# michal-szadkowski/rl-selfplay-mnk

Measured on AMD Instinct MI355X. Metric: env-steps/sec 9x9x5, 65536 parallel envs/GPU, random-policy rollout, higher is better.
Workload: dtype u64

## Files before the change

### rl-selfplay-mnk_amd/csrc/mnk_device.h

```cpp
#pragma once
#ifdef __HIPCC_RTC__
typedef unsigned char uint8_t;
typedef unsigned short uint16_t;
typedef unsigned int uint32_t;
typedef unsigned long long uint64_t;
typedef signed char int8_t;
typedef int int32_t;
typedef long long int64_t;
typedef unsigned long long uintptr_t;
#include "mnk_hip.h"
#else
#include <hip/hip_runtime.h>
#include <stdint.h>

#include "../../include/mnk_hip.h"
#endif

#define MNK_MAX_W 16
#define MNK_MAX_NW 32

struct MnkGeom {
  int m, n, k;
  int C;
  int W;
  int NW;
  int stride;
  uint32_t magic_n;
  uint32_t magic_stride;
  uint32_t magic_C;
  uint32_t magic_2C;
  uint32_t valid[MNK_MAX_NW];
};

__device__ __forceinline__ uint32_t mnk_div(uint32_t x, uint32_t magic) { return __umulhi(x, magic); }

__host__ __device__ inline bool aligned16(const void* p) { return (((uintptr_t)p) & 15u) == 0; }

struct MnkSample {
  const void* logits;
  int logits_dtype;
  const uint8_t* mask;
  uint64_t seed;
  const uint64_t* seed_dev;
  uint64_t step;
  const uint64_t* step_dev;
  int64_t env_id0;
  int deterministic;
  int64_t* actions;
  float* logp;
};

template <int CN>
__device__ __forceinline__ int geom_n(const MnkGeom& g) { return CN ? CN : g.n; }
template <int CK>
__device__ __forceinline__ int geom_k(const MnkGeom& g) { return CK ? CK : g.k; }

template <int CN>
__device__ __forceinline__ int mnk_bit_cell(const MnkGeom& g, uint32_t bit) {
  constexpr uint32_t magic = CN ? (uint32_t)((0x100000000ull + CN) / (uint32_t)(CN + 1)) : 0u;
  return (int)(bit - (CN ? __umulhi(bit, magic) : mnk_div(bit, g.magic_stride)));
}
template <int CN>
__device__ __forceinline__ uint32_t mnk_cell_bit(const MnkGeom& g, uint32_t cell) {
  return cell + (CN ? cell / (uint32_t)CN : mnk_div(cell, g.magic_n));
}

template <int NW>
__device__ __forceinline__ void bs_shr(uint32_t (&x)[NW], int s) {
  for (int q = s >> 5; q > 0; --q) {
#pragma unroll
    for (int w = 0; w < NW; ++w) x[w] = (w + 1 < NW) ? x[w + 1] : 0u;
  }
  const int r = s & 31;
  if (r) {
#pragma unroll
    for (int w = 0; w < NW; ++w) x[w] = __builtin_amdgcn_alignbit((w + 1 < NW) ? x[w + 1] : 0u, x[w], (uint32_t)r);
  }
}

template <int NW>
__device__ __forceinline__ void bs_shl(uint32_t (&x)[NW], int s) {
  for (int q = s >> 5; q > 0; --q) {
#pragma unroll
    for (int w = NW - 1; w >= 0; --w) x[w] = w > 0 ? x[w - 1] : 0u;
  }
  const int r = s & 31;
  if (r) {
#pragma unroll
    for (int w = NW - 1; w >= 0; --w) x[w] = __builtin_amdgcn_alignbit(x[w], w > 0 ? x[w - 1] : 0u, (uint32_t)(32 - r));
  }
}

template <int NW>
__device__ __forceinline__ bool bs_has_run(const uint32_t (&b)[NW], int d, int k) {
  uint32_t x[NW], t[NW];
#pragma unroll
  for (int w = 0; w < NW; ++w) x[w] = b[w];
  int len = 1;
  while (2 * len <= k) {
#pragma unroll
    for (int w = 0; w < NW; ++w) t[w] = x[w];
    bs_shr<NW>(t, len * d);
#pragma unroll
    for (int w = 0; w < NW; ++w) x[w] &= t[w];
    len *= 2;
  }
  if (len + 1 == k) {
#pragma unroll
    for (int w = 0; w < NW; ++w) t[w] = b[w];
    bs_shr<NW>(t, len * d);
#pragma unroll
    for (int w = 0; w < NW; ++w) x[w] &= t[w];
  } else if (len < k) {
#pragma unroll
    for (int w = 0; w < NW; ++w) t[w] = x[w];
    bs_shr<NW>(t, (k - len) * d);
#pragma unroll
    for (int w = 0; w < NW; ++w) x[w] &= t[w];
  }
  uint32_t any = 0;
#pragma unroll
  for (int w = 0; w < NW; ++w) any |= x[w];
  return any != 0;
}

template <int NW, int CN, int CK>
__device__ __forceinline__ bool mnk_plane_wins(const MnkGeom& g, const uint32_t (&b)[NW]) {
  const int n = geom_n<CN>(g), k = geom_k<CK>(g);
  bool hit = bs_has_run<NW>(b, 1, k);
  hit |= bs_has_run<NW>(b, n + 1, k);
  hit |= bs_has_run<NW>(b, n + 2, k);
  hit |= bs_has_run<NW>(b, n, k);
  return hit;
}

template <int NW, int CN, int CK>
__device__ __forceinline__ void mnk_plane_completions(const MnkGeom& g, const uint32_t (&plane)[NW],
                                                      const uint32_t (&empty)[NW], uint32_t (&out)[NW]) {
  const int n = geom_n<CN>(g), k = geom_k<CK>(g);
  constexpr int UK = CK ? CK : 1;
  uint32_t acc[NW];
#pragma unroll
  for (int w = 0; w < NW; ++w) acc[w] = 0u;
#pragma unroll
  for (int dir = 0; dir < 4; ++dir) {
    const int d = dir == 0 ? 1 : (dir == 1 ? n + 1 : (dir == 2 ? n + 2 : n));
    uint32_t lj[NW];
#pragma unroll
    for (int w = 0; w < NW; ++w) lj[w] = ~0u;
#pragma unroll UK
    for (int j = 0; j < k; ++j) {
      if (j > 0) {
        uint32_t t[NW];
#pragma unroll
        for (int w = 0; w < NW; ++w) t[w] = plane[w];
        bs_shl<NW>(t, j * d);
#pragma unroll
        for (int w = 0; w < NW; ++w) lj[w] &= t[w];
      }
      uint32_t rj[NW];
#pragma unroll
      for (int w = 0; w < NW; ++w) rj[w] = ~0u;
#pragma unroll UK
      for (int i = 1; i < k - j; ++i) {
        uint32_t t[NW];
#pragma unroll
        for (int w = 0; w < NW; ++w) t[w] = plane[w];
        bs_shr<NW>(t, i * d);
#pragma unroll
        for (int w = 0; w < NW; ++w) rj[w] &= t[w];
      }
#pragma unroll
      for (int w = 0; w < NW; ++w) acc[w] |= lj[w] & rj[w];
    }
  }
#pragma unroll
  for (int w = 0; w < NW; ++w) out[w] = acc[w] & empty[w];
}

#define MNK_SELECT_LEVEL(S)                        \
  "v_bfe_u32 %[t], %[x], %[pos], " #S "\n\t"       \
  "v_bcnt_u32_b32 %[t], %[t], %[nr]\n\t"          \
  "v_max_u32 %[nr], %[nr], %[t]\n\t"              \
  "v_ashrrev_i32 %[t], 31, %[t]\n\t"              \
  "v_and_or_b32 %[pos], %[t], " #S ", %[pos]\n\t"
__device__ __forceinline__ uint32_t select_bit32_nr(uint32_t x, uint32_t nr, uint32_t base) {
  uint32_t pos, t;
  asm("v_and_b32 %[t], 0xffff, %[x]\n\t"
      "v_bcnt_u32_b32 %[t], %[t], %[nr]\n\t"
      "v_max_u32 %[nr], %[nr], %[t]\n\t"
      "v_ashrrev_i32 %[t], 31, %[t]\n\t"
      "v_and_or_b32 %[pos], %[t], 16, %[base]\n\t"
      MNK_SELECT_LEVEL(8) MNK_SELECT_LEVEL(4) MNK_SELECT_LEVEL(2)
      "v_bfe_u32 %[t], %[x], %[pos], 1\n\t"
      "v_bitop3_b32 %[t], %[nr], %[t], %[t] bitop3:0x3f\n\t"
      "v_and_or_b32 %[pos], %[t], 1, %[pos]"
      : [pos] "=&v"(pos), [t] "=&v"(t), [nr] "+v"(nr)
      : [x] "v"(x), [base] "v"(base));
  return pos;
}
#undef MNK_SELECT_LEVEL

__device__ __forceinline__ int select_bit32(uint32_t x, int r) { return (int)select_bit32_nr(x, ~(uint32_t)r, 0u); }

template <int NW>
__device__ __forceinline__ int bs_popcount(const uint32_t (&x)[NW]) {
  int c = 0;
#pragma unroll
  for (int w = 0; w < NW; ++w) c += __popc(x[w]);
  return c;
}

template <int NW>
__device__ __forceinline__ int bs_select_hot(const uint32_t (&x)[NW], int r_, uint32_t (&hot)[NW]) {
  const uint32_t nr = ~(uint32_t)r_;
  uint32_t m[NW + 1], word = x[0], base = 0u, rank = nr, pre = 0u;
  m[0] = ~0u;
  m[NW] = 0u;
#pragma unroll
  for (int w = 1; w < NW; ++w) {
    pre += (uint32_t)__popc(x[w - 1]);
    const uint32_t t = pre + nr;
    m[w] = (uint32_t)((int32_t)t >> 31);
    rank = rank > t ? rank : t;
    word = __builtin_amdgcn_bitop3_b32(m[w], x[w], word, 0xca);
    base = __builtin_amdgcn_bitop3_b32(m[w], 32u * w, base, 0xca);
  }
  const uint32_t pos = select_bit32_nr(word, rank, base);
  const uint32_t one = 1u << (pos & 31u);
#pragma unroll
  for (int w = 0; w < NW; ++w) hot[w] = __builtin_amdgcn_bitop3_b32(one, m[w], m[w + 1], 0x40);
  return (int)pos;
}

template <int NW>
__device__ __forceinline__ int bs_select(const uint32_t (&x)[NW], int r) {
  uint32_t hot[NW];
  return bs_select_hot<NW>(x, r, hot);
}

struct Philox4 { uint32_t v[4]; };

__device__ __forceinline__ uint64_t mnk_mul_wide(uint32_t a, uint32_t m) {
  uint64_t product, carry;
  asm("v_mad_u64_u32 %0, %1, %2, %3, 0" : "=v"(product), "=s"(carry) : "v"(a), "s"(m));
  return product;
}

__device__ __forceinline__ Philox4 philox4x32_10(uint32_t c0, uint32_t c1, uint32_t c2, uint32_t c3,
                                                 uint32_t k0, uint32_t k1) {
  const uint32_t M0 = 0xD2511F53u, M1 = 0xCD9E8D57u;
#pragma unroll
  for (int r = 0; r < 10; ++r) {
    const uint64_t p0 = mnk_mul_wide(c0, M0), p1 = mnk_mul_wide(c2, M1);
    const uint32_t n0 = __builtin_amdgcn_bitop3_b32((uint32_t)(p1 >> 32), c1, k0, 0x96);
    const uint32_t n2 = __builtin_amdgcn_bitop3_b32((uint32_t)(p0 >> 32), c3, k1, 0x96);
    c0 = n0; c1 = (uint32_t)p1; c2 = n2; c3 = (uint32_t)p0;
    k0 += 0x9E3779B9u; k1 += 0xBB67AE85u;
  }
  Philox4 o;
  o.v[0] = c0; o.v[1] = c1; o.v[2] = c2; o.v[3] = c3;
  return o;
}

__device__ __forceinline__ Philox4 mnk_rng_block(uint64_t seed, uint64_t env, uint64_t q, uint32_t stream) {
  return philox4x32_10((uint32_t)env, (uint32_t)(env >> 32), (uint32_t)q,
                       stream | ((uint32_t)((q >> 32) & 0xFFFFFFu) << 8),
                       (uint32_t)seed, (uint32_t)(seed >> 32));
}

__device__ __forceinline__ uint32_t philox_word(const Philox4& b, uint32_t i) {
  uint32_t lo = (i & 1u) ? b.v[1] : b.v[0];
  uint32_t hi = (i & 1u) ? b.v[3] : b.v[2];
  return (i & 2u) ? hi : lo;
}

__device__ __forceinline__ uint32_t mnk_rand_u32(uint64_t seed, uint64_t env, uint64_t step, uint32_t stream) {
  Philox4 b = mnk_rng_block(seed, env, step >> 2, stream);
  return philox_word(b, (uint32_t)(step & 3));
}

template <int NW>
struct MnkEnv {
  uint32_t p[2][NW];
  uint32_t meta;
};

template <int NW, bool EXACT = false>
__device__ __forceinline__ void plane_load(uint32_t (&x)[NW], const uint64_t* plane, int64_t N, int W, int64_t i) {
#pragma unroll
  for (int q = 0; q < (NW + 1) / 2; ++q) {
    const uint64_t v = (EXACT || q < W) ? plane[(int64_t)q * N + i] : 0ull;
    x[2 * q] = (uint32_t)v;
    if (2 * q + 1 < NW) x[2 * q + 1] = (uint32_t)(v >> 32);
  }
}

template <int NW, bool EXACT = false>
__device__ __forceinline__ void plane_store(const uint32_t (&x)[NW], uint64_t* plane, int64_t N, int W, int64_t i) {
#pragma unroll
  for (int q = 0; q < (NW + 1) / 2; ++q) {
    const uint64_t hi = (2 * q + 1 < NW) ? (uint64_t)x[2 * q + 1] : 0ull;
    if (EXACT || q < W) plane[(int64_t)q * N + i] = (uint64_t)x[2 * q] | (hi << 32);
  }
}

template <int NW, bool EXACT = false>
__device__ __forceinline__ void rec_store(const uint32_t (&p0)[NW], const uint32_t (&p1)[NW], uint64_t* rows, int64_t N,
                                          int nw, int64_t i) {
#pragma unroll
  for (int w = 0; w < NW; ++w)
    if (EXACT || w < nw) rows[(int64_t)w * N + i] = (uint64_t)p0[w] | ((uint64_t)p1[w] << 32);
}

template <int NW, bool EXACT = false>
__device__ __forceinline__ void rec_load(uint32_t (&p0)[NW], uint32_t (&p1)[NW], const uint64_t* rows, int64_t N, int nw,
                                         int64_t i) {
#pragma unroll
  for (int w = 0; w < NW; ++w) {
    const uint64_t v = (EXACT || w < nw) ? rows[(int64_t)w * N + i] : 0ull;
    p0[w] = (uint32_t)v;
    p1[w] = (uint32_t)(v >> 32);
  }
}

template <int NW, bool EXACT = false>
__device__ __forceinline__ void env_load(MnkEnv<NW>& e, const uint64_t* planes, const uint32_t* meta, int64_t N,
                                         int W, int64_t i) {
  plane_load<NW, EXACT>(e.p[0], planes, N, W, i);
  plane_load<NW, EXACT>(e.p[1], planes + (int64_t)W * N, N, W, i);
  e.meta = meta[i];
}

template <int NW, bool EXACT = false>
__device__ __forceinline__ void env_store(const MnkEnv<NW>& e, uint64_t* planes, uint32_t* meta, int64_t N, int W,
                                          int64_t i) {
  plane_store<NW, EXACT>(e.p[0], planes, N, W, i);
  plane_store<NW, EXACT>(e.p[1], planes + (int64_t)W * N, N, W, i);
  meta[i] = e.meta;
}

template <int NW>
__device__ __forceinline__ void env_clear(MnkEnv<NW>& e) {
#pragma unroll
  for (int pl = 0; pl < 2; ++pl)
#pragma unroll
    for (int w = 0; w < NW; ++w) e.p[pl][w] = 0u;
  e.meta = 0u;
}

template <int NW>
__device__ __forceinline__ void env_legal(const MnkGeom& g, const MnkEnv<NW>& e, uint32_t (&legal)[NW]) {
#pragma unroll
  for (int w = 0; w < NW; ++w) legal[w] = ~(e.p[0][w] | e.p[1][w]) & g.valid[w];
}

template <int NW, int CN>
__device__ __forceinline__ int bs_pick_cell(const MnkGeom& g, uint32_t (&set)[NW], uint32_t x) {
  const int nl = bs_popcount<NW>(set);
#pragma unroll
  for (int w = 0; w < NW; ++w) set[w] = nl ? set[w] : g.valid[w];
  const int r = (int)__umulhi(x, (uint32_t)(nl ? nl : g.C));
  const uint32_t bit = (uint32_t)bs_select<NW>(set, r);
  return mnk_bit_cell<CN>(g, bit);
}

template <int NW, int CN>
__device__ __forceinline__ int env_pick_legal(const MnkGeom& g, const MnkEnv<NW>& e, uint32_t x) {
  uint32_t legal[NW];
  env_legal<NW>(g, e, legal);
  return bs_pick_cell<NW, CN>(g, legal, x);
}

template <int NW, int CN, int CK>
__device__ __forceinline__ void mnk_tactical_set(const MnkGeom& g, const uint32_t (&mine)[NW], const uint32_t (&theirs)[NW],
                                                 uint32_t (&set)[NW]) {
  uint32_t legal[NW], win[NW], block[NW];
#pragma unroll
  for (int w = 0; w < NW; ++w) legal[w] = ~(mine[w] | theirs[w]) & g.valid[w];
  mnk_plane_completions<NW, CN, CK>(g, mine, legal, win);
  mnk_plane_completions<NW, CN, CK>(g, theirs, legal, block);
  uint32_t any_win = 0, any_block = 0;
#pragma unroll
  for (int w = 0; w < NW; ++w) {
    any_win |= win[w];
    any_block |= block[w];
  }
#pragma unroll
  for (int w = 0; w < NW; ++w) set[w] = any_win ? win[w] : (any_block ? block[w] : legal[w]);
}

template <int NW, int CN, int CK>
__device__ __forceinline__ int env_pick_tactical(const MnkGeom& g, const MnkEnv<NW>& e, uint32_t x) {
  const uint32_t side = e.meta & 1u;
  uint32_t mine[NW], theirs[NW], set[NW];
#pragma unroll
  for (int w = 0; w < NW; ++w) {
    mine[w] = side ? e.p[1][w] : e.p[0][w];
    theirs[w] = side ? e.p[0][w] : e.p[1][w];
  }
  mnk_tactical_set<NW, CN, CK>(g, mine, theirs, set);
  return bs_pick_cell<NW, CN>(g, set, x);
}

struct MnkPly {
  bool win, done;
  int err;
};

template <int NW, int CN, int CK, bool TRUSTED = false>
__device__ __forceinline__ MnkPly env_play(const MnkGeom& g, MnkEnv<NW>& e, int64_t action, bool strict) {
  MnkPly out;
  out.win = false; out.done = false; out.err = 0;
  const int C = g.C;
  uint32_t a;
  if (TRUSTED) {
    a = (uint32_t)action;
  } else {
    const int64_t a64 = action < 0 ? action + C : action;
    if (a64 < 0 || a64 >= C) { out.err = 1; return out; }
    a = (uint32_t)a64;
  }
  const uint32_t bit = mnk_cell_bit<CN>(g, a);
  const int wsel = (int)(bit >> 5);
  const uint32_t one = 1u << (bit & 31u);
  const uint32_t side = e.meta & 1u;
  if (strict) {
    uint32_t occ = 0;
#pragma unroll
    for (int w = 0; w < NW; ++w) occ |= (w == wsel) ? ((e.p[0][w] | e.p[1][w]) & one) : 0u;
    if (occ) { out.err = 2; return out; }
  }
  uint32_t mine[NW];
#pragma unroll
  for (int w = 0; w < NW; ++w) {
    const uint32_t add = (w == wsel) ? one : 0u;
    e.p[0][w] |= side ? 0u : add;
    e.p[1][w] |= side ? add : 0u;
    mine[w] = side ? e.p[1][w] : e.p[0][w];
  }
  const uint32_t moves = (e.meta >> 1) + 1u;
  out.win = mnk_plane_wins<NW, CN, CK>(g, mine);
  const bool draw = (moves >= (uint32_t)C) && !out.win;
  out.done = out.win || draw;
  e.meta = (moves << 1) | (side ^ 1u);
  return out;
}

__device__ __forceinline__ void mnk_report(int32_t* err, int code, int64_t env) {
  if (err && atomicCAS(&err[0], 0, code) == 0) err[1] = (int32_t)env;
}
```

### rl-selfplay-mnk_amd/csrc/mnk_rollout_lane.h

```cpp
#pragma once
#include "mnk_device.h"
#include "mnk_pair_scan.h"

template <int NW, int CN, int CK, bool RECORD, int ACT = 0, bool PAIR = false, int WS = 1, bool SADDR = false>
struct RolloutLane {
  static constexpr bool EXACT = CN != 0;
  const MnkGeom& g;
  uint32_t cur[NW], oth[NW];
  uint32_t side, moves;
  int64_t N;
  uint32_t role = 0;
  uint32_t wrole = 0;
  uint32_t* vx = nullptr;
  uint64_t* rp = nullptr;
  uint32_t* rm = nullptr;
  static constexpr bool OFF32 = SADDR || PAIR;
  const char* rbase[OFF32 ? NW : 1] = {};
  const char* mbase = nullptr;
  uint32_t roff = 0, moff = 0;
  uint8_t* ra = nullptr;
  uint64_t quad = 0;
  uint32_t q32 = 0;
  uint8_t* rh = nullptr;
  uint32_t hi4 = 0, hiw = 0, hfill = 0;
  uint32_t lo = 0;
  uint32_t fill = 0;
  uint32_t acc_dw = 0, acc_white = 0;
  uint32_t moves_in = 0;
  uint32_t moves_parity = 0;

  __device__ __forceinline__ RolloutLane(const MnkGeom& g_, int64_t N_, int64_t i, uint64_t* rec_planes,
                                         uint32_t* rec_meta, void* act_log, uint32_t role_ = 0, uint32_t wrole_ = 0,
                                         uint32_t* vx_ = nullptr)
      : g(g_), N(N_), role(role_), wrole(wrole_), vx(vx_) {
    if (RECORD) {
      if (!PAIR) rp = rec_planes + i;
      rm = rec_meta + i;
      if (OFF32) {
#pragma unroll
        for (int w = 0; w < NW; ++w) rbase[w] = (const char*)(rec_planes + (int64_t)w * N);
        mbase = (const char*)rec_meta;
        roff = (uint32_t)i * 8u + (PAIR ? role * 4u : 0u);
        moff = (uint32_t)i * 4u;
      }
    }
    static_assert((ACT != 3 && ACT != 4) || (!PAIR && WS == 1), "the bit-packed action logs are built into the one-lane form only");
    if (ACT) ra = (uint8_t*)act_log + i * 4 * (ACT == 2 ? 2 : 1);
  }

  __device__ __forceinline__ void log_begin(void* act_log, int T, int64_t i) {
    if constexpr (ACT == 4) rh = (uint8_t*)act_log + ((int64_t)((T + 3) >> 2) * N + i) * 4;
  }

  __device__ __forceinline__ void load(const uint64_t* planes, const uint32_t* meta, int64_t i) {
    uint32_t p0[NW], p1[NW];
    plane_load<NW, EXACT>(p0, planes, N, g.W, i);
    plane_load<NW, EXACT>(p1, planes + (int64_t)g.W * N, N, g.W, i);
    const uint32_t mw = meta[i];
    side = mw & 1u;
    moves = moves_in = mw >> 1;
#pragma unroll
    for (int w = 0; w < NW; ++w) {
      cur[w] = side ? p1[w] : p0[w];
      oth[w] = side ? p0[w] : p1[w];
    }
  }

  __device__ __forceinline__ void store_planes(uint64_t* dst, int64_t i) const {
    uint32_t p0[NW], p1[NW];
#pragma unroll
    for (int w = 0; w < NW; ++w) {
      p0[w] = side ? oth[w] : cur[w];
      p1[w] = side ? cur[w] : oth[w];
    }
    plane_store<NW, EXACT>(p0, dst, N, g.W, i);
    plane_store<NW, EXACT>(p1, dst + (int64_t)g.W * N, N, g.W, i);
  }

  __device__ __forceinline__ void store_record() {
    if constexpr (PAIR) {
#pragma unroll
      for (int w = 0; w < NW; ++w)
        __builtin_nontemporal_store(role ? oth[w] : cur[w], (uint32_t*)(rbase[w] + (uint64_t)roff));
      roff += (uint32_t)NW * (uint32_t)N * 8u;
      return;
    }
    if constexpr (WS > 1) {
      static_assert(EXACT, "the waves-per-group form is built for the compile-time boards only");
#pragma unroll
      for (int r = 0; r < WS; ++r)
        if (wrole == (uint32_t)r) {
#pragma unroll
          for (int w = r * NW / WS; w < (r + 1) * NW / WS; ++w)
            __builtin_nontemporal_store((uint64_t)cur[w] | ((uint64_t)oth[w] << 32), rp + (int64_t)w * N);
        }
      rp += (int64_t)NW * N;
      return;
    }
    if constexpr (SADDR) {
#pragma unroll
      for (int w = 0; w < NW; ++w)
        if (EXACT || w < g.NW)
          __builtin_nontemporal_store((uint64_t)cur[w] | ((uint64_t)oth[w] << 32),
                                      (uint64_t*)(rbase[w] + (uint64_t)roff));
      roff += (uint32_t)g.NW * (uint32_t)N * 8u;
      return;
    }
#pragma unroll
    for (int w = 0; w < NW; ++w)
      if (EXACT || w < g.NW)
        __builtin_nontemporal_store((uint64_t)cur[w] | ((uint64_t)oth[w] << 32), rp + (int64_t)w * N);
    rp += (int64_t)g.NW * N;
  }

  __device__ __forceinline__ void store(uint64_t* planes, uint32_t* meta, int64_t i) const {
    if constexpr (PAIR) {
      uint32_t mine[NW];
#pragma unroll
      for (int w = 0; w < NW; ++w) mine[w] = (role ^ side) ? oth[w] : cur[w];
      plane_store<NW, EXACT>(mine, planes + (int64_t)role * g.W * N, N, g.W, i);
    } else {
      store_planes(planes, i);
    }
    meta[i] = (moves << 1) | side;
  }

  __device__ __forceinline__ void log_flush() {
    if constexpr (ACT == 3) {
      if (fill == 0u) {
        lo = q32;
        fill = 28u;
      } else {
        *(uint32_t*)ra = lo | (q32 << fill);
        ra += N * 4;
        lo = q32 >> (32u - fill);
        fill -= 4u;
      }
      q32 = 0;
      return;
    }
    if constexpr (ACT == 4) {
      *(uint32_t*)ra = q32;
      ra += N * 4;
      q32 = 0;
      hiw |= hi4 << hfill;
      hi4 = 0;
      hfill += 4u;
      if (hfill == 32u) {
        *(uint32_t*)rh = hiw;
        rh += N * 4;
        hiw = 0;
        hfill = 0;
      }
      return;
    }
    if (WS == 1 || wrole == 0) {
      if (ACT == 1) *(uint32_t*)ra = (uint32_t)quad;
      if (ACT == 2) *(uint64_t*)ra = quad;
    }
    ra += N * 4 * ACT;
    quad = 0;
  }

  __device__ __forceinline__ void log_finish(int T) {
    if (ACT && (T & 3)) log_flush();
    if constexpr (ACT == 3) {
      if (fill) *(uint32_t*)ra = lo;
    }
    if constexpr (ACT == 4) {
      if (hfill) *(uint32_t*)rh = hiw;
    }
  }

  template <bool FAST = false>
  __device__ __forceinline__ int pick(uint32_t x, uint32_t (&hot)[NW], uint32_t& nlegal) const {
    uint32_t legal[NW];
#pragma unroll
    for (int w = 0; w < NW; ++w) legal[w] = ~(cur[w] | oth[w]) & g.valid[w];
    const int nl = bs_popcount<NW>(legal);
    nlegal = (uint32_t)nl;
    int n = nl;
    if (!FAST && __builtin_amdgcn_ballot_w64(nl == 0) != 0) {
#pragma unroll
      for (int w = 0; w < NW; ++w) legal[w] = nl ? legal[w] : g.valid[w];
      n = nl ? nl : g.C;
    }
    const int r = (int)__umulhi(x, (uint32_t)n);
    const uint32_t bit = (uint32_t)bs_select_hot<NW>(legal, r, hot);
    return mnk_bit_cell<CN>(g, bit);
  }

  template <bool FAST = false>
  __device__ __forceinline__ void ply(uint32_t x, int field) {
    uint32_t hot[NW];
    uint32_t nlegal;
    const int a = pick<FAST>(x, hot, nlegal);
    if constexpr (ACT == 3) {
      q32 |= (uint32_t)a << (7 * field);
      if (field == 3) log_flush();
    } else if constexpr (ACT == 4) {
      q32 |= ((uint32_t)a & 0xFFu) << (8 * field);
      hi4 |= ((uint32_t)a >> 8) << field;
      if (field == 3) log_flush();
    } else if (ACT) {
      quad |= (uint64_t)(uint32_t)a << (8 * ACT * field);
      if (field == 3) log_flush();
    }
    ply_hot<FAST>(a, hot, nlegal);
  }

  __device__ __forceinline__ void ply_action(int a) {
    ply_bit(a, mnk_cell_bit<CN>(g, (uint32_t)a));
  }

  __device__ __forceinline__ void ply_bit(int a, uint32_t bit) {
    const int wsel = (int)(bit >> 5);
    const uint32_t one = 1u << (bit & 31u);
    uint32_t hot[NW];
#pragma unroll
    for (int w = 0; w < NW; ++w) hot[w] = (w == wsel) ? one : 0u;
    ply_hot<false>(a, hot);
  }

  template <bool FAST = false>
  __device__ __forceinline__ void ply_hot(int a, const uint32_t (&hot)[NW], uint32_t nlegal = 0) {
    if (RECORD) store_record();
#pragma unroll
    for (int w = 0; w < NW; ++w) cur[w] |= hot[w];
    if (!FAST) ++moves;
    uint32_t win;
    if constexpr (PAIR) {
      uint32_t hit = bs_run_bits_pair<NW, CK, CN + 1, CN + 2>(cur, role) | bs_run_bits_pair<NW, CK, 1, CN>(cur, role);
      hit |= pair_swap(hit);
      win = hit ? 1u : 0u;
    } else if constexpr (WS > 1) {
      bool hit = false;
      if constexpr (WS == 4) {
        if (wrole == 0) hit = bs_has_run<NW>(cur, 1, CK);
        else if (wrole == 1) hit = bs_has_run<NW>(cur, CN + 1, CK);
        else if (wrole == 2) hit = bs_has_run<NW>(cur, CN + 2, CK);
        else hit = bs_has_run<NW>(cur, CN, CK);
      } else {
        if (wrole == 0) hit = bs_has_run<NW>(cur, 1, CK) | bs_has_run<NW>(cur, CN + 1, CK);
        else hit = bs_has_run<NW>(cur, CN + 2, CK) | bs_has_run<NW>(cur, CN, CK);
      }
      uint32_t* slot = vx + ((moves_parity & 1u) * 64u + (threadIdx.x & 63u)) * WS;
      slot[wrole] = hit ? 1u : 0u;
      asm volatile("s_waitcnt lgkmcnt(0)\n\ts_barrier" ::: "memory");
      uint32_t any = 0;
#pragma unroll
      for (int r = 0; r < WS; ++r) any |= slot[r];
      win = any;
      ++moves_parity;
    } else {
      win = mnk_plane_wins<NW, CN, CK>(g, cur) ? 1u : 0u;
    }
    const uint32_t done = win | ((FAST ? nlegal == 1u : moves >= (uint32_t)g.C) ? 1u : 0u);
    if (RECORD) {
      const uint32_t mword = (uint32_t)a | (win << MNK_REC_REWARD_SHIFT) | (done << MNK_REC_DONE_BIT) | (side << MNK_REC_SIDE_BIT);
      if constexpr (OFF32) {
        __builtin_nontemporal_store(mword, (uint32_t*)(mbase + (uint64_t)moff));
        moff += (uint32_t)N * 4u;
      } else {
        if (WS == 1 || wrole == WS - 1) __builtin_nontemporal_store(mword, rm);
        rm += N;
      }
    }
    acc_dw += done | (win << 16);
    acc_white += win & side;
#pragma unroll
    for (int w = 0; w < NW; ++w) {
      const uint32_t c = cur[w];
      cur[w] = done ? 0u : oth[w];
      oth[w] = done ? 0u : c;
    }
    side = done ? 0u : (side ^ 1u);
    if (!FAST) moves = done ? 0u : moves;
  }

  __device__ __forceinline__ uint32_t acc_done() const { return acc_dw & 0xFFFFu; }
  __device__ __forceinline__ uint32_t acc_win() const { return acc_dw >> 16; }

  __device__ __forceinline__ bool consistent() const {
    uint32_t occ[NW];
#pragma unroll
    for (int w = 0; w < NW; ++w) occ[w] = cur[w] | oth[w];
    return (uint32_t)bs_popcount<NW>(occ) == moves && moves < (uint32_t)g.C;
  }

  __device__ __forceinline__ void finish_fast() {
    uint32_t occ[NW];
#pragma unroll
    for (int w = 0; w < NW; ++w) occ[w] = cur[w] | oth[w];
    moves = (uint32_t)bs_popcount<NW>(occ);
  }
};

template <bool FAST, typename Lane>
__device__ __forceinline__ void rollout_plies(Lane& L, int T, uint64_t seed, uint64_t step0, uint64_t env) {
  int t = 0;
  uint64_t step = step0;
  if (step & 3) {
    const Philox4 blk = mnk_rng_block(seed, env, step >> 2, MNK_STREAM_MOVE);
    for (; t < T && (step & 3); ++t, ++step)
      L.template ply<FAST>(philox_word(blk, (uint32_t)(step & 3)), (int)(step & 3));
  }
  for (; t + 4 <= T; t += 4, step += 4) {
    const Philox4 blk = mnk_rng_block(seed, env, step >> 2, MNK_STREAM_MOVE);
    L.template ply<FAST>(blk.v[0], 0);
    L.template ply<FAST>(blk.v[1], 1);
    L.template ply<FAST>(blk.v[2], 2);
    L.template ply<FAST>(blk.v[3], 3);
  }
  if (t < T) {
    const Philox4 blk = mnk_rng_block(seed, env, step >> 2, MNK_STREAM_MOVE);
    for (uint32_t j = 0; t < T; ++t, ++j) L.template ply<FAST>(philox_word(blk, j), (int)j);
  }
}

template <int NW, int CN, int CK, bool RECORD, int ACT, bool SADDR = false>
__device__ __forceinline__ void rollout_random_body(const MnkGeom& g, uint64_t* planes, uint32_t* meta, int64_t N, int T,
                                                    uint64_t seed, uint64_t step0, int64_t env_id0,
                                                    uint64_t* rec_planes, uint32_t* rec_meta, unsigned long long* stats,
                                                    void* act_log) {
  __shared__ unsigned int lds_stats[MNK_STATS_COUNTERS];
  if (threadIdx.x < MNK_STATS_COUNTERS) lds_stats[threadIdx.x] = 0u;
  __syncthreads();
  const int64_t i = (int64_t)blockIdx.x * blockDim.x + threadIdx.x;
  if (i < N) {
    RolloutLane<NW, CN, CK, RECORD, ACT, false, 1, SADDR> L(g, N, i, rec_planes, rec_meta, act_log);
    L.log_begin(act_log, T, i);
    L.load(planes, meta, i);
    const uint64_t env = (uint64_t)(env_id0 + i);
    constexpr bool TRY_FAST = NW <= 3 || (NW == 6 && CN == 13);
    if (TRY_FAST && __builtin_amdgcn_ballot_w64(!L.consistent()) == 0) {
      rollout_plies<true>(L, T, seed, step0, env);
      L.finish_fast();
    } else {
      rollout_plies<false>(L, T, seed, step0, env);
    }
    L.log_finish(T);
    L.store(planes, meta, i);
    if (stats) {
      const uint32_t len_sum = L.moves_in + (uint32_t)T - L.moves;
      if (L.acc_done()) atomicAdd(&lds_stats[0], L.acc_done());
      if (L.acc_win() - L.acc_white) atomicAdd(&lds_stats[1], L.acc_win() - L.acc_white);
      if (L.acc_white) atomicAdd(&lds_stats[2], L.acc_white);
      if (L.acc_done() - L.acc_win()) atomicAdd(&lds_stats[3], L.acc_done() - L.acc_win());
      if (len_sum) atomicAdd(&lds_stats[4], len_sum);
    }
  }
  __syncthreads();
  if (stats && threadIdx.x < MNK_STATS_COUNTERS && lds_stats[threadIdx.x])
    atomicAdd(&stats[(size_t)(blockIdx.x % MNK_STATS_REPLICAS) * MNK_STATS_STRIDE + threadIdx.x],
              (unsigned long long)lds_stats[threadIdx.x]);
}

template <bool FAST, typename Lane>
__device__ __forceinline__ void pair_plies(Lane& L, int T, uint64_t seed, uint64_t step0, uint64_t env, uint32_t role) {
  int t = 0;
  uint64_t step = step0;
  for (; t < T && (step & 7); ++t, ++step)
    L.template ply<FAST>(mnk_rand_u32(seed, env, step, MNK_STREAM_MOVE), (int)(step & 3));
  for (; t + 8 <= T; t += 8, step += 8) {
    const Philox4 mine = mnk_rng_block(seed, env, (step >> 2) + role, MNK_STREAM_MOVE);
    uint32_t lo[4], hi[4];
#pragma unroll
    for (int j = 0; j < 4; ++j) {
      const uint32_t other = pair_swap(mine.v[j]);
      lo[j] = role ? other : mine.v[j];
      hi[j] = role ? mine.v[j] : other;
    }
#pragma unroll
    for (int j = 0; j < 4; ++j) L.template ply<FAST>(lo[j], j);
#pragma unroll
    for (int j = 0; j < 4; ++j) L.template ply<FAST>(hi[j], j);
  }
  for (; t < T; ++t, ++step) L.template ply<FAST>(mnk_rand_u32(seed, env, step, MNK_STREAM_MOVE), (int)(step & 3));
}

template <int NW, int CN, int CK, bool RECORD, int ACT>
__device__ __forceinline__ void rollout_random_pair_body(const MnkGeom& g, uint64_t* planes, uint32_t* meta, int64_t N, int T,
                                                         uint64_t seed, uint64_t step0, int64_t env_id0, uint64_t* rec_planes,
                                                         uint32_t* rec_meta, unsigned long long* stats, void* act_log) {
  __shared__ unsigned int lds_stats[MNK_STATS_COUNTERS];
  if (threadIdx.x < MNK_STATS_COUNTERS) lds_stats[threadIdx.x] = 0u;
  __syncthreads();
  const uint32_t role = threadIdx.x & 1u;
  const int64_t i = (int64_t)blockIdx.x * 32 + (threadIdx.x >> 1);
  if (i < N) {
    RolloutLane<NW, CN, CK, RECORD, ACT, true> L(g, N, i, rec_planes, rec_meta, act_log, role);
    L.load(planes, meta, i);
    const uint64_t env = (uint64_t)(env_id0 + i);
    constexpr bool TRY_FAST = NW <= 3;
    if (TRY_FAST && __builtin_amdgcn_ballot_w64(!L.consistent()) == 0) {
      pair_plies<true>(L, T, seed, step0, env, role);
      L.finish_fast();
    } else {
      pair_plies<false>(L, T, seed, step0, env, role);
    }
    if (ACT && (T & 3)) L.log_flush();
    L.store(planes, meta, i);
    if (stats && role == 0) {
      const uint32_t len_sum = L.moves_in + (uint32_t)T - L.moves;
      if (L.acc_done()) atomicAdd(&lds_stats[0], L.acc_done());
      if (L.acc_win() - L.acc_white) atomicAdd(&lds_stats[1], L.acc_win() - L.acc_white);
      if (L.acc_white) atomicAdd(&lds_stats[2], L.acc_white);
      if (L.acc_done() - L.acc_win()) atomicAdd(&lds_stats[3], L.acc_done() - L.acc_win());
      if (len_sum) atomicAdd(&lds_stats[4], len_sum);
    }
  }
  __syncthreads();
  if (stats && threadIdx.x < MNK_STATS_COUNTERS && lds_stats[threadIdx.x])
    atomicAdd(&stats[(size_t)(blockIdx.x % MNK_STATS_REPLICAS) * MNK_STATS_STRIDE + threadIdx.x],
              (unsigned long long)lds_stats[threadIdx.x]);
}

template <int NW, int CN, int CK, bool RECORD, int ACTB>
__device__ __forceinline__ void replay_actions_body(const MnkGeom& g, uint64_t* planes, uint32_t* meta, int64_t N, int T,
                                                    const void* act_log, uint64_t* rec_planes, uint32_t* rec_meta,
                                                    int32_t* err) {
  const int64_t i = (int64_t)blockIdx.x * blockDim.x + threadIdx.x;
  if (i >= N) return;
  RolloutLane<NW, CN, CK, RECORD> L(g, N, i, rec_planes, rec_meta, nullptr);
  L.load(planes, meta, i);
  if constexpr (ACTB == 3) {
    bool bad7 = false;
    auto play7 = [&](uint32_t a) {
      if (a >= (uint32_t)g.C) { bad7 = true; a = 0; }
      L.ply_action((int)a);
    };
    const int quads = (T + 3) >> 2, nwords = (7 * quads + 7) >> 3;
    const uint32_t* src = (const uint32_t*)act_log + i;
    uint32_t ahead = nwords ? src[0] : 0u;
    int w = 1;
    uint32_t cur = 0, have = 0;
    auto take_word = [&]() -> uint32_t {
      const uint32_t word = ahead;
      ahead = src[(int64_t)(w < nwords ? w : nwords - 1) * N];
      ++w;
      return word;
    };
    auto next_quad = [&]() -> uint32_t {
      uint32_t q;
      if (have == 28u) {
        q = cur;
        cur = 0u;
        have = 0u;
      } else {
        const uint32_t word = take_word();
        q = (cur | (word << have)) & 0x0FFFFFFFu;
        cur = word >> (28u - have);
        have += 4u;
      }
      return q;
    };
    int t = 0;
    for (; t + 4 <= T; t += 4) {
      const uint32_t q = next_quad();
      play7(q & 0x7Fu);
      play7((q >> 7) & 0x7Fu);
      play7((q >> 14) & 0x7Fu);
      play7((q >> 21) & 0x7Fu);
    }
    if (t < T) {
      uint32_t q = next_quad();
      for (; t < T; ++t, q >>= 7) play7(q & 0x7Fu);
    }
    if (bad7) mnk_report(err, MNK_ERR_ACTION_RANGE, i);
    L.store(planes, meta, i);
    return;
  }
  if constexpr (ACTB == 4) {
    bool bad9 = false;
    auto play9 = [&](uint32_t a) {
      if (a >= (uint32_t)g.C) { bad9 = true; a = 0; }
      L.ply_action((int)a);
    };
    const int quads = (T + 3) >> 2, hwords = (T + 31) >> 5;
    const uint32_t* lo = (const uint32_t*)act_log + i;
    const uint32_t* hi = lo + (int64_t)quads * N;
    uint32_t ahead = quads ? lo[0] : 0u;
    uint32_t hbits = hwords ? hi[0] : 0u;
    int t = 0;
    for (int q = 0; t < T; ++q) {
      const uint32_t word = ahead;
      ahead = lo[(int64_t)(q + 1 < quads ? q + 1 : q) * N];
      if (q && (q & 7) == 0) hbits = hi[(int64_t)(q >> 3) * N];
      const uint32_t h4 = hbits >> (4 * (q & 7));
      if (t + 4 <= T) {
        play9((word & 0xFFu) | ((h4 & 1u) << 8));
        play9(((word >> 8) & 0xFFu) | ((h4 & 2u) << 7));
        play9(((word >> 16) & 0xFFu) | ((h4 & 4u) << 6));
        play9((word >> 24) | ((h4 & 8u) << 5));
        t += 4;
      } else {
        for (int j = 0; t < T; ++t, ++j) play9(((word >> (8 * j)) & 0xFFu) | (((h4 >> j) & 1u) << 8));
      }
    }
    if (bad9) mnk_report(err, MNK_ERR_ACTION_RANGE, i);
    L.store(planes, meta, i);
    return;
  }
  constexpr uint32_t FIELD = ACTB == 1 ? 0xFFu : 0xFFFFu;
  auto fetch = [&](int q) -> uint64_t {
    if (ACTB == 1) return (uint64_t)((const uint32_t*)act_log)[(int64_t)q * N + i];
    return ((const uint64_t*)act_log)[(int64_t)q * N + i];
  };
  bool bad = false;
  auto play = [&](uint32_t a) {
    if (a >= (uint32_t)g.C) { bad = true; a = 0; }
    L.ply_action((int)a);
  };
  const int words = (T + 3) >> 2;
  uint64_t ahead = words ? fetch(0) : 0;
  int t = 0;
  for (int q = 0; t + 4 <= T; ++q, t += 4) {
    const uint64_t quad = ahead;
    ahead = fetch(q + 1 < words ? q + 1 : q);
    play((uint32_t)(quad >> (0 * 8 * ACTB)) & FIELD);
    play((uint32_t)(quad >> (1 * 8 * ACTB)) & FIELD);
    play((uint32_t)(quad >> (2 * 8 * ACTB)) & FIELD);
    play((uint32_t)(quad >> (3 * 8 * ACTB)) & FIELD);
  }
  for (uint64_t quad = ahead; t < T; ++t, quad >>= 8 * ACTB) play((uint32_t)quad & FIELD);
  if (bad) mnk_report(err, MNK_ERR_ACTION_RANGE, i);
  L.store(planes, meta, i);
}


template <int NW, int CN, int CK, bool RECORD, int ACT, bool SADDR = false>
__global__ void __launch_bounds__(64)
k_rollout_random(MnkGeom g, uint64_t* planes, uint32_t* meta, int64_t N, int T, uint64_t seed, uint64_t step0,
                 int64_t env_id0, uint64_t* rec_planes, uint32_t* rec_meta, unsigned long long* stats,
                 void* act_log) {
  rollout_random_body<NW, CN, CK, RECORD, ACT, SADDR>(g, planes, meta, N, T, seed, step0, env_id0, rec_planes, rec_meta,
                                                      stats, act_log);
}

template <int NW, int CN, int CK, bool RECORD, int ACT>
__global__ void __launch_bounds__(64)
k_rollout_random_pair(MnkGeom g, uint64_t* planes, uint32_t* meta, int64_t N, int T, uint64_t seed, uint64_t step0,
                      int64_t env_id0, uint64_t* rec_planes, uint32_t* rec_meta, unsigned long long* stats,
                      void* act_log) {
  rollout_random_pair_body<NW, CN, CK, RECORD, ACT>(g, planes, meta, N, T, seed, step0, env_id0, rec_planes, rec_meta, stats,
                                                    act_log);
}

template <int NW, int CN, int CK, bool RECORD, int ACTB>
__global__ void __launch_bounds__(64)
k_replay_actions(MnkGeom g, uint64_t* planes, uint32_t* meta, int64_t N, int T, const void* act_log,
                 uint64_t* rec_planes, uint32_t* rec_meta, int32_t* err) {
  replay_actions_body<NW, CN, CK, RECORD, ACTB>(g, planes, meta, N, T, act_log, rec_planes, rec_meta, err);
}
```

Measured before the change: 203.8 billion.

## Interleave next Philox block rounds with current plies in rollout loop

Splits the Philox 10-round generator into a resumable state object and, for exact-geometry small boards, computes the next block's rounds in slices interleaved between the four plies that consume the current block. This is meant to hide RNG latency behind the ply logic and give the scheduler independent instructions to overlap. In exchange it keeps an extra Philox state live, which raises register pressure, and it computes one surplus block at the end of the loop.

```diff
diff --git a/rl-selfplay-mnk_amd/csrc/mnk_device.h b/rl-selfplay-mnk_amd/csrc/mnk_device.h
--- a/rl-selfplay-mnk_amd/csrc/mnk_device.h
+++ b/rl-selfplay-mnk_amd/csrc/mnk_device.h
@@ -247,26 +247,48 @@
   return product;
 }
 
+struct PhiloxRun {
+  uint32_t c0, c1, c2, c3, k0, k1;
+
+  template <int R>
+  __device__ __forceinline__ void rounds() {
+    const uint32_t M0 = 0xD2511F53u, M1 = 0xCD9E8D57u;
+#pragma unroll
+    for (int r = 0; r < R; ++r) {
+      const uint64_t p0 = mnk_mul_wide(c0, M0), p1 = mnk_mul_wide(c2, M1);
+      const uint32_t n0 = __builtin_amdgcn_bitop3_b32((uint32_t)(p1 >> 32), c1, k0, 0x96);
+      const uint32_t n2 = __builtin_amdgcn_bitop3_b32((uint32_t)(p0 >> 32), c3, k1, 0x96);
+      c0 = n0; c1 = (uint32_t)p1; c2 = n2; c3 = (uint32_t)p0;
+      k0 += 0x9E3779B9u; k1 += 0xBB67AE85u;
+    }
+  }
+
+  __device__ __forceinline__ Philox4 block() const {
+    Philox4 o;
+    o.v[0] = c0; o.v[1] = c1; o.v[2] = c2; o.v[3] = c3;
+    return o;
+  }
+};
+
+__device__ __forceinline__ PhiloxRun mnk_rng_begin(uint64_t seed, uint64_t env, uint64_t q, uint32_t stream) {
+  PhiloxRun p;
+  p.c0 = (uint32_t)env; p.c1 = (uint32_t)(env >> 32); p.c2 = (uint32_t)q;
+  p.c3 = stream | ((uint32_t)((q >> 32) & 0xFFFFFFu) << 8);
+  p.k0 = (uint32_t)seed; p.k1 = (uint32_t)(seed >> 32);
+  return p;
+}
+
 __device__ __forceinline__ Philox4 philox4x32_10(uint32_t c0, uint32_t c1, uint32_t c2, uint32_t c3,
                                                  uint32_t k0, uint32_t k1) {
-  const uint32_t M0 = 0xD2511F53u, M1 = 0xCD9E8D57u;
-#pragma unroll
-  for (int r = 0; r < 10; ++r) {
-    const uint64_t p0 = mnk_mul_wide(c0, M0), p1 = mnk_mul_wide(c2, M1);
-    const uint32_t n0 = __builtin_amdgcn_bitop3_b32((uint32_t)(p1 >> 32), c1, k0, 0x96);
-    const uint32_t n2 = __builtin_amdgcn_bitop3_b32((uint32_t)(p0 >> 32), c3, k1, 0x96);
-    c0 = n0; c1 = (uint32_t)p1; c2 = n2; c3 = (uint32_t)p0;
-    k0 += 0x9E3779B9u; k1 += 0xBB67AE85u;
-  }
-  Philox4 o;
-  o.v[0] = c0; o.v[1] = c1; o.v[2] = c2; o.v[3] = c3;
-  return o;
+  PhiloxRun p{c0, c1, c2, c3, k0, k1};
+  p.template rounds<10>();
+  return p.block();
 }
 
 __device__ __forceinline__ Philox4 mnk_rng_block(uint64_t seed, uint64_t env, uint64_t q, uint32_t stream) {
-  return philox4x32_10((uint32_t)env, (uint32_t)(env >> 32), (uint32_t)q,
-                       stream | ((uint32_t)((q >> 32) & 0xFFFFFFu) << 8),
-                       (uint32_t)seed, (uint32_t)(seed >> 32));
+  PhiloxRun p = mnk_rng_begin(seed, env, q, stream);
+  p.template rounds<10>();
+  return p.block();
 }
 
 __device__ __forceinline__ uint32_t philox_word(const Philox4& b, uint32_t i) {
diff --git a/rl-selfplay-mnk_amd/csrc/mnk_rollout_lane.h b/rl-selfplay-mnk_amd/csrc/mnk_rollout_lane.h
--- a/rl-selfplay-mnk_amd/csrc/mnk_rollout_lane.h
+++ b/rl-selfplay-mnk_amd/csrc/mnk_rollout_lane.h
@@ -296,7 +296,7 @@
   }
 };
 
-template <bool FAST, typename Lane>
+template <bool FAST, bool AHEAD, typename Lane>
 __device__ __forceinline__ void rollout_plies(Lane& L, int T, uint64_t seed, uint64_t step0, uint64_t env) {
   int t = 0;
   uint64_t step = step0;
@@ -305,16 +305,35 @@
     for (; t < T && (step & 3); ++t, ++step)
       L.template ply<FAST>(philox_word(blk, (uint32_t)(step & 3)), (int)(step & 3));
   }
-  for (; t + 4 <= T; t += 4, step += 4) {
-    const Philox4 blk = mnk_rng_block(seed, env, step >> 2, MNK_STREAM_MOVE);
-    L.template ply<FAST>(blk.v[0], 0);
-    L.template ply<FAST>(blk.v[1], 1);
-    L.template ply<FAST>(blk.v[2], 2);
-    L.template ply<FAST>(blk.v[3], 3);
-  }
-  if (t < T) {
-    const Philox4 blk = mnk_rng_block(seed, env, step >> 2, MNK_STREAM_MOVE);
-    for (uint32_t j = 0; t < T; ++t, ++j) L.template ply<FAST>(philox_word(blk, j), (int)j);
+  if constexpr (AHEAD) {
+    if (t < T) {
+      Philox4 blk = mnk_rng_block(seed, env, step >> 2, MNK_STREAM_MOVE);
+      for (; t + 4 <= T; t += 4, step += 4) {
+        PhiloxRun next = mnk_rng_begin(seed, env, (step + 4) >> 2, MNK_STREAM_MOVE);
+        next.template rounds<1>();
+        L.template ply<FAST>(blk.v[0], 0);
+        next.template rounds<3>();
+        L.template ply<FAST>(blk.v[1], 1);
+        next.template rounds<3>();
+        L.template ply<FAST>(blk.v[2], 2);
+        next.template rounds<3>();
+        L.template ply<FAST>(blk.v[3], 3);
+        blk = next.block();
+      }
+      for (uint32_t j = 0; t < T; ++t, ++j) L.template ply<FAST>(philox_word(blk, j), (int)j);
+    }
+  } else {
+    for (; t + 4 <= T; t += 4, step += 4) {
+      const Philox4 blk = mnk_rng_block(seed, env, step >> 2, MNK_STREAM_MOVE);
+      L.template ply<FAST>(blk.v[0], 0);
+      L.template ply<FAST>(blk.v[1], 1);
+      L.template ply<FAST>(blk.v[2], 2);
+      L.template ply<FAST>(blk.v[3], 3);
+    }
+    if (t < T) {
+      const Philox4 blk = mnk_rng_block(seed, env, step >> 2, MNK_STREAM_MOVE);
+      for (uint32_t j = 0; t < T; ++t, ++j) L.template ply<FAST>(philox_word(blk, j), (int)j);
+    }
   }
 }
 
@@ -333,11 +352,12 @@
     L.load(planes, meta, i);
     const uint64_t env = (uint64_t)(env_id0 + i);
     constexpr bool TRY_FAST = NW <= 3 || (NW == 6 && CN == 13);
+    constexpr bool AHEAD = CN != 0 && NW <= 3;
     if (TRY_FAST && __builtin_amdgcn_ballot_w64(!L.consistent()) == 0) {
-      rollout_plies<true>(L, T, seed, step0, env);
+      rollout_plies<true, AHEAD>(L, T, seed, step0, env);
       L.finish_fast();
     } else {
-      rollout_plies<false>(L, T, seed, step0, env);
+      rollout_plies<false, AHEAD>(L, T, seed, step0, env);
     }
     L.log_finish(T);
     L.store(planes, meta, i);
```

Result: no change. 203.5 billion (-0.1%).
